# dfm/george

Hardware: AMD Instinct MI355X
Metric: gp_compute_plus_log_likelihood_effective_tflops (higher is better)
Workload: dtype f64; 1 GPU; N=65536 1-D sorted uniform(0,10) x, var(y)*ExpSquaredKernel(1.0), yerr=0.1, dense Cholesky fp64 (BasicSolver path): compute()+log_likelihood(); N=65536, kernel=ExpSquared, solver=dense-cholesky, parallelism=1gpu

## Files before the change

george_amd/_native.py:

```python
import ctypes as C
import os

import numpy as np

_HERE = os.path.dirname(os.path.abspath(__file__))
LIB_PATH = os.path.join(_HERE, "csrc", "libgeorge_amd.so")

GH_MAX_AXES, GH_MAX_NDIM, GH_MAX_PARAMS, GH_MAX_METRIC = 8, 16, 4, 36
GH_MAX_NODES, GH_MAX_GRAD, GH_MAX_STACK = 64, 64, 8
GH_OK, GH_ERR_NOT_PD, GH_ERR_BAD_ARG, GH_ERR_HIP, GH_ERR_NOT_COMPUTED, GH_ERR_DIM, GH_ERR_NOMEM, GH_ERR_RANK, GH_REFACTORIZE = range(9)
GH_OP_LEAF, GH_OP_SUM, GH_OP_PRODUCT = 0, 1, 2


class gh_knode(C.Structure):
    _fields_ = [
        ("op", C.c_int32), ("kernel_type", C.c_int32), ("metric_type", C.c_int32),
        ("ndim", C.c_int32), ("naxes", C.c_int32), ("blocked", C.c_int32),
        ("n_params", C.c_int32), ("n_metric", C.c_int32),
        ("axes", C.c_int32 * GH_MAX_AXES),
        ("params", C.c_double * GH_MAX_PARAMS),
        ("constant", C.c_double),
        ("metric", C.c_double * GH_MAX_METRIC),
        ("min_block", C.c_double * GH_MAX_AXES),
        ("max_block", C.c_double * GH_MAX_AXES),
# ... 63 lines not shown

_vp, _dp, _i64, _i32 = C.c_void_p, C.c_void_p, C.c_int64, C.c_int32

SIGNATURES = {
    "gh_device_count": (C.c_int, []),
    "gh_last_error": (C.c_char_p, []),
    "gh_version": (C.c_char_p, []),
    "gh_release_caches": (None, [C.c_int32]),
    "gh_set_cache_limit": (None, [C.c_int64]),
    "gh_microbench_mfma_f64": (C.c_int, [C.POINTER(C.c_double)]),
    "gh_microbench_hbm_copy": (C.c_int, [C.POINTER(C.c_double)]),
    "gh_debug_set_mfma": (C.c_int, [C.c_int]),
    "gh_debug_set_gemm_sp": (C.c_int, [C.c_int]),
    "gh_debug_set_adaptive_panels": (C.c_int, [C.c_int]),
    "gh_debug_set_update_group": (C.c_int, [C.c_int]),
    "gh_debug_set_update_hide": (C.c_double, [C.c_double]),
    "gh_debug_chol_plan": (C.c_int, [C.c_int64, C.c_int64, C.c_int64, C.c_int32, C.c_double, C.POINTER(C.c_int64), C.c_int32, C.POINTER(C.c_int32),
                                     C.POINTER(C.c_int64), C.c_int32, C.POINTER(C.c_int32), C.POINTER(C.c_int32)]),
    "gh_debug_set_build_on_chain": (C.c_int, [C.c_int]),
    "gh_debug_set_append_path": (C.c_int, [C.c_int]),
    "gh_debug_set_remove_path": (C.c_int, [C.c_int]),
    "gh_debug_check_remove_args": (C.c_int, [_i64, _dp, _i64]),
    "gh_debug_set_gemm_grouped": (C.c_int, [C.c_int]),
    "gh_debug_set_hodlr_passes": (C.c_int, [C.c_int]),
    "gh_debug_set_hodlr_leaf_gj": (C.c_int, [C.c_int]),
    "gh_debug_set_hodlr_wave_aca": (C.c_int, [C.c_int]),
    "gh_debug_set_hodlr_coop_wgs": (C.c_int, [C.c_int]),
    "gh_debug_set_hodlr_coop_lower": (C.c_int, [C.c_int]),
    "gh_debug_set_hodlr_lpt": (C.c_int, [C.c_int]),
    "gh_debug_set_hodlr_u_from_v": (C.c_int, [C.c_int]),
    "gh_debug_set_hodlr_core_fused": (C.c_int, [C.c_int]),
    "gh_debug_set_hodlr_coop_singles": (C.c_int, [C.c_int]),
    "gh_debug_set_hodlr_leaf_fused": (C.c_int, [C.c_int]),
    "gh_debug_set_hodlr_strip_cols": (C.c_int, [C.c_int]),
    "gh_debug_stream_overlap": (C.c_int, [_vp, C.POINTER(C.c_double), C.c_int]),
    "gh_debug_stream_dispatch": (C.c_int, [_vp, C.POINTER(C.c_double), C.c_int]),
    "gh_microbench_suite": (C.c_int, [C.POINTER(C.c_double), C.c_int]),
    "gh_microbench_mfma_f64_ceiling": (C.c_int, [C.POINTER(C.c_double), C.c_int]),
    "gh_kernel_create": (C.c_int, [C.POINTER(gh_knode), C.c_int, C.POINTER(_vp)]),
    "gh_kernel_destroy": (None, [_vp]),
    "gh_kernel_ndim": (C.c_int, [_vp]),
    "gh_kernel_size": (C.c_int, [_vp]),
    "gh_kernel_value_general": (C.c_int, [_vp, _dp, _i64, _dp, _i64, _dp]),
    "gh_kernel_value_symmetric": (C.c_int, [_vp, _dp, _i64, _dp]),
    "gh_kernel_value_diagonal": (C.c_int, [_vp, _dp, _dp, _i64, _dp]),
    "gh_kernel_gradient_general": (C.c_int, [_vp, _dp, _dp, _i64, _dp, _i64, _dp]),
# ... 160 lines not shown
```

george_amd/csrc/gh_chol.hip:

```cpp
#include <math.h>
#include <chrono>
#include "gh_chol_impl.h"
#include "../../include/george_amd_debug.h"

__global__ __launch_bounds__(256) void potf2_inv_kernel(double* A, long lda, double* dinv,
                                                        long long* info, long long base) {
  __shared__ double s[T * LP];
  __shared__ int fail_at;
  const int tid = threadIdx.x;
  if (*info != 0) return;
  if (tid == 0) fail_at = -1;
  for (int idx = tid; idx < T * T; idx += 256) {
    const int i = idx >> 7, j = idx & 127;
    s[i * LP + j] = A[(long)i * lda + j];
  }
  __syncthreads();
  const int ty = tid >> 4, tx = tid & 15;
  for (int j = 0; j < T; ++j) {
    const double d = s[j * LP + j];
    if (!(d > 0.0)) {
      if (tid == 0) fail_at = j;
      break;
    }
    const double ajj = sqrt(d);
// ... 238 lines not shown
  *st = s->st;
  *bufs = s->batch;
  return GH_OK;
}
extern "C" int gh_chol_get_update_intervals(const gh_chol* s, double* out, int32_t max_launches, int32_t* n_out) {
  if (!s || !n_out || (max_launches > 0 && !out)) { gh_set_error("null argument"); return GH_ERR_BAD_ARG; }
  const int32_t have = (int32_t)(s->upd_intervals.size() / 3);
  *n_out = have;
  for (int32_t i = 0; i < have && i < max_launches; ++i)
    for (int q = 0; q < 3; ++q) out[3 * i + q] = s->upd_intervals[3 * (size_t)i + q];
  return GH_OK;
}
extern "C" int gh_chol_get_profile(const gh_chol* s, gh_chol_profile* out) {
  if (!s || !out) { gh_set_error("null argument"); return GH_ERR_BAD_ARG; }
  *out = s->prof;
  return GH_OK;
}

static inline double* blk(double* A, int64_t ld, int64_t r, int64_t c) { return A + r * ld + c; }

static thread_local bool t_gemm_small_lds = false;
struct SmallLdsGuard { bool prev; explicit SmallLdsGuard(bool v) : prev(t_gemm_small_lds) { t_gemm_small_lds = v; } ~SmallLdsGuard() { t_gemm_small_lds = prev; } };
int gh_gemm_nt(hipStream_t st, double* C, int64_t ldc, const double* A, int64_t lda, const double* B, int64_t ldb,
               int64_t M, int64_t N, int64_t K, double alpha, double beta, bool lower) {
  GhGemm g = gemm_desc(C, ldc, A, lda, true, B, ldb, true, M, N, K, alpha, beta);
  g.small_lds = t_gemm_small_lds;
  g.lower = lower;
  return gh_launch_gemm(g, st);
}

static bool use_simple_potf2() {
  static int v = -1;
  if (v < 0) { const char* e = getenv("GEORGE_AMD_POTF2"); v = (e && e[0] == 's') ? 1 : 0; }
  return v == 1;
}

int gh_chol_potrf_block(hipStream_t st, double* A, int64_t ld, int64_t n, double* dinv, long long* d_info, long long base) {
  for (int64_t j0 = 0; j0 < n; j0 += T) {
    double* dj = dinv + (j0 / T) * T * T;
    if (use_simple_potf2()) {
      hipLaunchKernelGGL(potf2_inv_kernel, dim3(1), dim3(256), 0, st, blk(A, ld, j0, j0), (long)ld, dj, d_info, base + j0);
      GH_HIP(hipGetLastError());
    } else {
      GH_CHECK(gh_launch_potf2_mfma(blk(A, ld, j0, j0), ld, dj, d_info, base + j0, st));
    }
    const int64_t rem = n - (j0 + T);
    if (rem > 0) {
      double* P = blk(A, ld, j0 + T, j0);
      GH_CHECK(gh_gemm_nt(st, P, ld, P, ld, dj, T, rem, T, T, 1.0, 0.0, false));
      GH_CHECK(gh_gemm_nt(st, blk(A, ld, j0 + T, j0 + T), ld, P, ld, P, ld, rem, rem, T, -1.0, 1.0, true));
// ... 186 lines not shown
    if (prev) GH_HIP(hipStreamWaitEvent(sp, prev, 0));
    GH_CHECK(narrow(sp, j, j + 1));
    const int last_near = std::min(j + depth, P - 1);
    if (j + 2 <= last_near || (depth >= 2 && j + 2 <= P - 1)) GH_HIP(hipStreamWaitEvent(sn, s->ev_p[j], 0));
    for (int c = j + 2; c <= last_near; ++c) {
      if (c == j + depth && j >= 1) GH_HIP(hipStreamWaitEvent(sn, s->ev_w[j - 1], 0));
      GH_CHECK(narrow(sn, j, c));
      if (c == j + 2) GH_HIP(hipEventRecord(s->ev_nf[j], sn));
    }
    if (depth >= 2 && j + 2 > last_near) GH_HIP(hipEventRecord(s->ev_nf[j], sn));
    const int cw = j + depth + 1;
    hipStream_t sw = wide_stream(j);
    if (sw_prev && sw_prev != sw && j >= 1) GH_HIP(hipStreamWaitEvent(sw, s->ev_w[j - 1], 0));
    sw_prev = sw;
    GH_HIP(hipStreamWaitEvent(sw, s->ev_p[j], 0));
    if (cw <= P - 1) {
      const int64_t kw = c0(cw), m2 = np - kw;
      const long et = prof ? s->next_ev() : -1;
      if (et >= 0) {
        GH_HIP(hipEventRecord(s->ev_pool[et].a, sw)); s->ev_trailing.push_back((size_t)et); s->ev_update.push_back((size_t)et);
        s->ev_update_flops.push_back((double)(m2 / T) * (m2 / T + 1) / 2.0 * 2.0 * T * T * (double)nbc(j));
      }
      const double* P2 = blk(A, ld, kw, c0(j));
      GH_CHECK(gh_gemm_nt(sw, blk(A, ld, kw, kw), ld, P2, ld, P2, ld, m2, m2, nbc(j), -1.0, 1.0, true));
      if (et >= 0) GH_HIP(hipEventRecord(s->ev_pool[et].b, sw));
      const double tiles = (double)(m2 / T) * (m2 / T + 1) / 2.0;
      s->prof.trailing_flops += tiles * 2.0 * T * T * (double)nbc(j);
      s->prof.update_flops += tiles * 2.0 * T * T * (double)nbc(j);
      s->prof.n_trailing += 1;
    }
    GH_HIP(hipEventRecord(s->ev_w[j], sw));
  }
  const bool join_on_chain = !s->shared_streams || gh_shared_main_crowded(s->opts.device);
  if (sm != s->st && join_on_chain) {
    GH_HIP(hipEventRecord(s->ev_sync[2], sn));
    GH_HIP(hipStreamWaitEvent(sp, s->ev_sync[2], 0));
    GH_HIP(hipEventRecord(s->ev_xfer, sm));
    GH_HIP(hipStreamWaitEvent(sp, s->ev_xfer, 0));
    if (P >= 2) GH_HIP(hipStreamWaitEvent(sp, s->ev_w[P - 2], 0));
    s->tail = sp;
    return GH_OK;
  }
  GH_HIP(hipEventRecord(s->ev_sync[1], sp));
  GH_HIP(hipStreamWaitEvent(s->st, s->ev_sync[1], 0));
  GH_HIP(hipEventRecord(s->ev_sync[2], sn));
  GH_HIP(hipStreamWaitEvent(s->st, s->ev_sync[2], 0));
  if (sm != s->st) {
// ... 253 lines not shown
```

george_amd/csrc/gh_chol_impl.h:

```cpp
#pragma once
#include <string.h>
#include <algorithm>
#include <vector>
#include "gh_common.h"
#include "gh_chol_plan.h"

#define T 128
#define LP 129
#define CHAIN_THREADS 512

struct EvPair { hipEvent_t a, b; };

struct gh_chol {
  gh_chol_opts opts;
  hipStream_t st = nullptr;
  hipStream_t st2 = nullptr;
  hipStream_t st3 = nullptr;
  bool shared_streams = false;
  hipStream_t st4 = nullptr;
  hipEvent_t ev_diag[32] = {};
  hipEvent_t ev_aux = nullptr, ev_aux2 = nullptr;
  std::vector<hipEvent_t> ev_p, ev_w, ev_nf;
  GhCholPlan plan;
  std::vector<hipEvent_t> ev_plan;
// ... 54 lines not shown
static inline unsigned* fwd_flags(const gh_chol* s) { return (unsigned*)s->chain.p; }
static inline unsigned* bwd_flags(const gh_chol* s) { return (unsigned*)s->chain.p + (s->np / T + 1); }
static inline int* fwd_fail(const gh_chol* s) { return (int*)(fwd_flags(s) + s->np / T); }
static inline int* bwd_fail(const gh_chol* s) { return (int*)(bwd_flags(s) + s->np / T); }
static inline int* append_fail(const gh_chol* s) { return (int*)s->chain.p; }

static inline int read_scalars(const gh_chol* s, double* host, int count, hipStream_t st) {
  GH_HIP(hipMemcpyAsync(host, s->scal.d(), (size_t)count * sizeof(double), hipMemcpyDeviceToHost, st));
  return GH_OK;
}
static inline long long info_from_bits(double word) { long long info = 0; memcpy(&info, &word, sizeof(long long)); return info; }

static inline GhGemm gemm_desc(double* C, int64_t ldc, const double* A, int64_t lda, bool a_km, const double* B, int64_t ldb, bool b_km,
                               int64_t M, int64_t N, int64_t K, double alpha, double beta) {
  GhGemm g{};
  g.C = C; g.ldc = ldc; g.A = A; g.lda = lda; g.B = B; g.ldb = ldb; g.M = M; g.N = N; g.K = K;
  g.alpha = alpha; g.beta = beta; g.a_km = a_km; g.b_km = b_km;
  return g;
}

int gh_chol_set_device(gh_chol* s);
int gh_chol_need_computed(gh_chol* s);
int gh_gemm_nt(hipStream_t st, double* C, int64_t ldc, const double* A, int64_t lda, const double* B, int64_t ldb,
               int64_t M, int64_t N, int64_t K, double alpha, double beta, bool lower);
int gh_chol_potrf_block(hipStream_t st, double* A, int64_t ld, int64_t n, double* dinv, long long* d_info, long long base);
struct ComputeCtx { long e_all = -1, e_build = -1; };
int gh_chol_compute_enqueue(gh_chol* s, gh_kernel* k, const double* x, int64_t n, int32_t ndim, const double* yerr, ComputeCtx& c);
int gh_chol_compute_finish(gh_chol* s, const ComputeCtx& c, double ld_host, long long info_host, double* logdet_out);

int gh_launch_potf2_mfma(double* A, int64_t lda, double* dinv, long long* info, long long base, hipStream_t st);

int gh_launch_logdet(const double* A, long lda, long n, double* out, double* part, hipStream_t st);
int gh_launch_logdet_accum(const double* A, long lda, long n, double* out, hipStream_t st);
int gh_chol_linv(hipStream_t st, const double* L, const double* dinv, int64_t np, double* Linv);
int gh_launch_trsv_fwd_chain(const double* L, long ld, const double* dinv, int64_t nt, const double* w, double* z, unsigned* flags, hipStream_t st);
int gh_launch_trsv_bwd_chain(const double* L, long ld, const double* dinv, int64_t nt, const double* w, double* x, unsigned* flags, hipStream_t st);
int gh_launch_trsv_fwd_chain_rows(const double* L, long ld, const double* dinv, int64_t nt0, const double* Y, long ldy, double* Z, long ldz,
                                  int64_t m, bool multi, int* fail, hipStream_t st);
int gh_chain_timeout(const char* who, bool forward_failed, bool backward_failed);
```

george_amd/csrc/gh_common.h:

```cpp
#pragma once
#include <hip/hip_runtime.h>
#include <stdint.h>
#include <stdio.h>
#include <functional>
#include <mutex>
#include <string>
#include <vector>
#include "../../include/george_amd.h"
#include "gh_eval.h"

#define GH_TILE 128

void gh_set_error(const char* fmt, ...);

#define GH_HIP(expr)                                                                   \
  do {                                                                                 \
    hipError_t e_ = (expr);                                                            \
    if (e_ != hipSuccess) {                                                            \
      gh_set_error("HIP error %d (%s) at %s:%d: %s", (int)e_, hipGetErrorString(e_),   \
                   __FILE__, __LINE__, #expr);                                         \
      return GH_ERR_HIP;                                                               \
    }                                                                                  \
  } while (0)

// ... 130 lines not shown
int gh_lgo_gram_chunks(int64_t n, int nslots, int64_t* rows_per);
int gh_launch_lgo_gram(const double* Linv, int64_t np, int64_t n, const GhLgoSlots& t, double* part, double* Cs, hipStream_t st);
int gh_launch_lgo_gather(const double* Kinv, int64_t np, const GhLgoSlots& t, double* Cs, hipStream_t st);
int gh_launch_lgo_slots(const double* R, const double* Rinv, const GhLgoSlots& t, const double* alpha, double* resid, double* var,
                        double* u_pt, double* lpd, double* cov, double* Ws, hipStream_t st);
int gh_launch_lgo_block_scale(const double* Kinv, int64_t np, int64_t n, const GhLgoSlots& t, const double* Tm, double* S,
                              hipStream_t st);

int gh_launch_potf2_batched(double* A, int64_t lda, int64_t stride_a, double* dinv, int64_t stride_d, long long* info,
                            int nbatch, hipStream_t st);

struct GhGemm {
  double* C; int64_t ldc;
  const double* A; int64_t lda;
  const double* B; int64_t ldb;
  int64_t M, N, K;
  double alpha, beta;
  bool a_km, b_km;
  bool lower;
  bool klo_max;
  bool khi_col;
  bool khi_row;
  bool small_lds;
  int stair_n = 0;
  int64_t stair_rows = 0;
  const int64_t* stair_cols = nullptr;
};
#define GH_GEMM_STAIR_MAX 128
int gh_launch_gemm(const GhGemm& g, hipStream_t st);

int gh_stage_points(const double* xs, int64_t m, int ndim, GhBuf& own, hipStream_t st, const double** xs_dev);
int gh_copy_rows(double* dst, int64_t ldd, const double* src, int64_t lds, int64_t cols, int64_t rows, bool from_caller, hipStream_t st);
int gh_launch_colreduce(const double* A, const double* z, const double* P, const double* Q, int64_t ld, int64_t nrows, int64_t rows_per,
                        int64_t nchunks, int64_t cols, double* pmu, double* pvar, int64_t ldp, double* mu, double* var, int threads,
                        hipStream_t st);
typedef std::function<int(const double* sK, double* sSecond, int64_t ld, int64_t np, int cw, size_t strip_bytes)> GhMakeSecond;
int gh_predict_strips(gh_kernel* k, const double* x, int64_t n, int ndim, const double* alpha, const double* xs_dev, int64_t m,
                      int64_t strip_cols, int64_t red_rows, int64_t red_chunks, double* mu, double* var, double* cov, hipStream_t st,
                      bool first_second, const GhMakeSecond& make_second);
struct GhPstrf {
  double* A; int64_t lda, stride_a;
  int64_t m, nbatch;
  double tol; const double* tol_dev;
  double* L; int64_t ldl, stride_l;
  int64_t rows_l, cols_l;
  long long* piv; long long* rank;
  double* resid;
  void* work; size_t work_bytes;
};
size_t gh_pstrf_work_bytes(int64_t m, int64_t nbatch);
int gh_launch_pstrf(const GhPstrf& p, hipStream_t st);
struct GhSample {
// ... 19 lines not shown
```

george_amd/csrc/gh_gemm.hip:

```cpp
#include <stdlib.h>
#include <algorithm>
#include "gh_common.h"
#include "../../include/george_amd_debug.h"

#include "gh_gemm_tile.h"

#ifndef GH_GEMM_SP_DEFAULT
#define GH_GEMM_SP_DEFAULT 1
#endif

struct GemmDev {
  double* C; long ldc;
  const double* A; long lda;
  const double* B; long ldb;
  long K;
  double alpha, beta;
  int tiles_m, tiles_n;
  int lower, klo_max, khi_col, khi_row;
  long nblk;
  int preload;
  int prio;
  int grouped;
  int stair_n, stair_h;
  unsigned stair_pre[GH_GEMM_STAIR_MAX + 1];
};

__device__ __forceinline__ long xcd_remap(long bid, long nblk) {
  const long q = nblk / 8, r = nblk % 8;
  const long xcd = bid % 8, idx = bid / 8;
  return (xcd < r ? xcd * (q + 1) : r * (q + 1) + (xcd - r) * q) + idx;
}

#ifndef GH_TILE_GROUP
#define GH_TILE_GROUP 8
#endif
__device__ __forceinline__ void grouped_rect(long l, int rows, int cols, int& tm, int& tn) {
  constexpr int G = GH_TILE_GROUP;
  const int g = (int)(l / ((long)G * cols));
  const int gg = min(G, rows - g * G);
  const long r = l - (long)g * G * cols;
  tn = (int)(r / gg);
  tm = g * G + (int)(r % gg);
}
__device__ __forceinline__ void grouped_tri(long l, int T, int& tm, int& tn) {
  constexpr int G = GH_TILE_GROUP;
  constexpr long H = (long)G * (G + 1) / 2;
  long g = (long)((sqrt(((double)H - 0.5 * G * G) * ((double)H - 0.5 * G * G) + 2.0 * G * G * (double)l) - ((double)H - 0.5 * G * G)) /
                  ((double)G * G));
  auto start = [&](long q) { return (long)G * G * q * (q - 1) / 2 + q * H; };
  while (start(g) > l) --g;
  while (start(g + 1) <= l) ++g;
  const int r0 = (int)g * G, gg = min(G, T - r0);
  long r = l - start(g);
  const long rect = (long)gg * (r0 + 1);
  if (r < rect) {
    tn = (int)(r / gg);
    tm = r0 + (int)(r % gg);
    return;
  }
  r -= rect;
  int j = 1;
  while (r >= gg - j) { r -= gg - j; ++j; }
  tn = r0 + j;
  tm = r0 + j + (int)r;
}
__device__ __forceinline__ bool tile_of(const GemmDev& g, int& tm, int& tn) {
  const bool rowmajor = !g.grouped;
  if (g.stair_n) {
    const long ls = xcd_remap(blockIdx.x, g.nblk);
    int s = 0;
    while (s + 1 < g.stair_n && ls >= (long)g.stair_pre[s + 1]) ++s;
    const int r = (int)(ls - (long)g.stair_pre[s]);
    tn = r / g.stair_h;
    tm = (g.stair_n - 1 - s) * g.stair_h + r % g.stair_h;
    return true;
  }
  const long l = (g.klo_max | g.khi_col | g.khi_row) ? (long)blockIdx.x : xcd_remap(blockIdx.x, g.nblk);
  if (g.lower) {
    const long tri = (long)g.tiles_n * (g.tiles_n + 1) / 2;
    if (l < tri) {
      if (!rowmajor) {
        grouped_tri(l, g.tiles_n, tm, tn);
      } else {
        long t = (long)((sqrt(8.0 * (double)l + 1.0) - 1.0) * 0.5);
        while (t * (t + 1) / 2 > l) --t;
        while ((t + 1) * (t + 2) / 2 <= l) ++t;
        tm = (int)t;
        tn = (int)(l - t * (t + 1) / 2);
      }
    } else if (!rowmajor) {
      grouped_rect(l - tri, g.tiles_m - g.tiles_n, g.tiles_n, tm, tn);
      tm += g.tiles_n;
    } else {
      tm = g.tiles_n + (int)((l - tri) / g.tiles_n);
      tn = (int)((l - tri) % g.tiles_n);
    }
  } else if (!rowmajor) {
    grouped_rect(l, g.tiles_m, g.tiles_n, tm, tn);
  } else {
    tm = (int)(l / g.tiles_n);
    tn = (int)(l % g.tiles_n);
  }
  return true;
}

template <bool KM>
__device__ __forceinline__ void stage_load(const double* base, long ld, long r0, long k0, int tid, double2 (&v)[4]) {
  if (KM) {
    const int row = tid >> 3, kc = (tid & 7) * 2;
#pragma unroll
    for (int i = 0; i < 4; ++i)
      v[i] = *reinterpret_cast<const double2*>(base + (r0 + row + 32 * i) * ld + k0 + kc);
  } else {
    const int k = tid >> 6, m = (tid & 63) * 2;
#pragma unroll
    for (int i = 0; i < 4; ++i)
      v[i] = *reinterpret_cast<const double2*>(base + (k0 + k + 4 * i) * ld + r0 + m);
  }
}
template <bool KM>
__device__ __forceinline__ void stage_store(double* s, int tid, const double2 (&v)[4]) {
  if (KM) {
    const int row = tid >> 3, kc = (tid & 7) * 2;
#pragma unroll
    for (int i = 0; i < 4; ++i)
// ... 112 lines not shown
    for (int i = 0; i < 4; ++i)
#pragma unroll
      for (int j = 0; j < 4; ++j)
        acc[i][j] = __builtin_amdgcn_mfma_f64_16x16x4f64(a[0][i], b[0][j], acc[i][j], 0, 0, 0);
    __builtin_amdgcn_sched_barrier(0);
    if (kt + 1 < nk) {
      if (cur) { GH_DMA_ISSUE(oa, sA[0]) GH_DMA_ISSUE(ob, sB[0]) }
      else     { GH_DMA_ISSUE(oa, sA[1]) GH_DMA_ISSUE(ob, sB[1]) }
    }
    __builtin_amdgcn_sched_barrier(0);
#pragma unroll
    for (int kk = 1; kk < 4; ++kk)
#pragma unroll
      for (int i = 0; i < 4; ++i)
#pragma unroll
        for (int j = 0; j < 4; ++j)
          acc[i][j] = __builtin_amdgcn_mfma_f64_16x16x4f64(a[kk][i], b[kk][j], acc[i][j], 0, 0, 0);
    __builtin_amdgcn_sched_barrier(0);
    __syncthreads();
  }
  gemm_epilogue(g, acc, row0 + wm * 64, col0 + wn * 64, fr, fk);
}

template <bool LOWER>
__global__ __launch_bounds__(256, 2) void gemm_f64_mfma_dma_sp(GemmDev g) {
  __shared__ __attribute__((aligned(1024))) double sm[4 * BM * BK];
  double* const sA0 = sm; double* const sA1 = sm + BM * BK;
  double* const sB0 = sm + 2 * BM * BK; double* const sB1 = sm + 3 * BM * BK;
  int tm, tn;
  if (!tile_of(g, tm, tn)) return;
  if (g.prio) __builtin_amdgcn_s_setprio(3);
  const long row0 = (long)tm * BM, col0 = (long)tn * BN;
  const int tid = threadIdx.x, lane = tid & 63, wave = __builtin_amdgcn_readfirstlane(tid >> 6);
  const int wm = wave >> 1, wn = wave & 1;
  const int fr = lane & 15, fk = lane >> 4;
  v4d acc[4][4];
  const long nk = g.K / BK;
  DmaOperand<true> oa, ob;
  oa.init(g.A, g.lda, row0, 0, wave, lane, wm);
  ob.init(g.B, g.ldb, col0, 0, wave, lane, wn);
  const int dst = wave * 4 * 128;
  const unsigned lbase = (unsigned)(unsigned long)(gh_lds_void*)sm;
  const unsigned pa0 = lbase + (unsigned)(oa.f0 + oa.off2[0]) * 8u, pa1 = lbase + (unsigned)(oa.f0 + oa.off2[1]) * 8u;
  const unsigned pb0 = lbase + 2u * BM * BK * 8u + (unsigned)(ob.f0 + ob.off2[0]) * 8u;
  const unsigned pb1 = lbase + 2u * BM * BK * 8u + (unsigned)(ob.f0 + ob.off2[1]) * 8u;
  constexpr int B1 = BM * BK * 8;
  v2d a01[4], b01[4], a23[4], b23[4];

  GH_DMA_ISSUE(oa, sA0) GH_DMA_ISSUE(ob, sB0)
  gemm_init_acc(g, acc, row0 + wm * 64, col0 + wn * 64, fr, fk);
  __syncthreads();
// ... 283 lines not shown
extern "C" int gh_debug_set_mfma(int mode) {
  const int prev = mfma_mode();
  g_mfma = mode == 0 ? 0 : 1;
  return prev;
}

static int g_gemm_sp = -1;
static int gemm_sp_mode() {
  if (g_gemm_sp < 0) g_gemm_sp = GH_GEMM_SP_DEFAULT;
  return g_gemm_sp;
}
static int g_gemm_grouped = -1;
extern "C" int gh_debug_set_gemm_grouped(int mode) {
  const int prev = g_gemm_grouped;
  g_gemm_grouped = mode < 0 ? -1 : (mode != 0);
  return prev;
}
extern "C" int gh_debug_set_gemm_sp(int mode) {
  const int prev = gemm_sp_mode();
  g_gemm_sp = mode < 0 ? GH_GEMM_SP_DEFAULT : (mode != 0);
  return prev;
}

int gh_launch_gemm(const GhGemm& h, hipStream_t st) {
  if (h.M <= 0 || h.N <= 0) return GH_OK;
  if (h.M % BM || h.N % BN || h.K % BK) { gh_set_error("gemm: sizes must be multiples of the tile (%ld %ld %ld)", (long)h.M, (long)h.N, (long)h.K); return GH_ERR_BAD_ARG; }
  if (h.lower && h.M < h.N) { gh_set_error("gemm: lower needs M >= N (a lower trapezoid: the leading N columns of a lower-triangular C)"); return GH_ERR_BAD_ARG; }
  GemmDev g;
  g.C = h.C; g.ldc = h.ldc; g.A = h.A; g.lda = h.lda; g.B = h.B; g.ldb = h.ldb; g.K = h.K;
  g.alpha = h.alpha; g.beta = h.beta;
  g.tiles_m = (int)(h.M / BM); g.tiles_n = (int)(h.N / BN);
  g.lower = h.lower; g.klo_max = h.klo_max; g.khi_col = h.khi_col; g.khi_row = h.khi_row;
  g.nblk = h.lower ? (long)g.tiles_n * (g.tiles_n + 1) / 2 + (long)(g.tiles_m - g.tiles_n) * g.tiles_n : (long)g.tiles_m * g.tiles_n;
  g.stair_n = 0; g.stair_h = 0;
  if (h.stair_n > 0) {
    g.stair_n = h.stair_n; g.stair_h = (int)(h.stair_rows / BM);
    g.tiles_m = g.stair_n * g.stair_h; g.tiles_n = (int)(h.stair_cols[h.stair_n - 1] / BN);
    long at = 0;
    for (int s = 0; s < h.stair_n; ++s) { g.stair_pre[s] = (unsigned)at; at += (long)g.stair_h * (h.stair_cols[h.stair_n - 1 - s] / BN); }
    g.stair_pre[h.stair_n] = (unsigned)at;
    g.nblk = at;
  }
  g.prio = g.nblk <= 512 ? 1 : 0;
  g.grouped = (!(h.klo_max | h.khi_col | h.khi_row) && (long)h.N * h.K * 8 > (128L << 20)) ? 1 : 0;
  if (g_gemm_grouped >= 0 && !(h.klo_max | h.khi_col | h.khi_row)) g.grouped = g_gemm_grouped;
  g.preload = (h.beta != 0.0 && (h.beta == h.alpha || h.beta == -h.alpha)) ? 1 : 0;
  if (g.nblk > 0x7fffffffL) { gh_set_error("gemm: grid too large"); return GH_ERR_BAD_ARG; }
  const dim3 grid((unsigned)g.nblk), block(256);
  const int mode = mfma_mode();
#define GH_GEMM_LAUNCH(AK, BKM) hipLaunchKernelGGL((gemm_f64_valu<AK, BKM>), grid, block, 0, st, g)
  constexpr int64_t GH_DMA_MAX_LD = ((1LL << 31) - 4096) / (128 * 8);
  const bool dma = mode == 1 && h.lda % 2 == 0 && h.ldb % 2 == 0 && h.lda <= GH_DMA_MAX_LD && h.ldb <= GH_DMA_MAX_LD &&
                   ((uintptr_t)h.A % 16) == 0 && ((uintptr_t)h.B % 16) == 0;
#define GH_DMA_LAUNCH(AK, BKM)                                                                            \
  do {                                                                                                   \
    if (h.lower) hipLaunchKernelGGL((gemm_f64_mfma_dma<AK, BKM, true>), grid, block, 0, st, g);          \
    else         hipLaunchKernelGGL((gemm_f64_mfma_dma<AK, BKM, false>), grid, block, 0, st, g);         \
  } while (0)
  const bool inplace = (const double*)h.C == h.A || (const double*)h.C == h.B;
  if (dma && !h.stair_n && h.a_km && h.b_km && h.K == 128 && g.nblk <= 128 && !h.klo_max && !h.khi_col && !h.khi_row && !h.small_lds &&
      (!inplace || ((const double*)h.C == h.A && (const double*)h.C != h.B && h.N == 128 && !h.lower))) {
    GemmDev q = g;
    if (inplace) {
      q.tiles_m = (int)(h.M / 16); q.tiles_n = 1;
      q.nblk = q.tiles_m;
      hipLaunchKernelGGL((gemm_f64_mfma_k128<1, 4, 1, 2>), dim3((unsigned)q.nblk), block, 0, st, q);
    } else {
      q.tiles_m = (int)(h.M / 64); q.tiles_n = (int)(h.N / 64);
      q.nblk = (long)q.tiles_m * q.tiles_n;
      hipLaunchKernelGGL((gemm_f64_mfma_k128<2, 2, 2, 2>), dim3((unsigned)q.nblk), block, 0, st, q);
    }
    GH_HIP(hipGetLastError());
    return GH_OK;
  }
  if (dma && !h.stair_n && h.a_km && h.b_km && g.nblk <= 128 && !h.klo_max && !h.khi_col && !h.khi_row && (!h.lower || h.M == h.N) &&
      (!inplace || (h.N == 128 && !h.lower))) {
    GemmDev q = g;
    if (inplace) {
      q.tiles_m = (int)(h.M / 64); q.tiles_n = 1;
      q.nblk = q.tiles_m;
      hipLaunchKernelGGL(gemm_f64_mfma_dma64<4>, dim3((unsigned)q.nblk), block, 0, st, q);
    } else {
      q.tiles_m = (int)(h.M / 64); q.tiles_n = (int)(h.N / 64);
      q.nblk = h.lower ? 4 * g.nblk : (long)q.tiles_m * q.tiles_n;
      hipLaunchKernelGGL(gemm_f64_mfma_dma64<2>, dim3((unsigned)q.nblk), block, 0, st, q);
    }
  }
  else if (dma && h.a_km && h.b_km && gemm_sp_mode() && !h.klo_max && !h.khi_col && !h.khi_row && h.K % (2 * BK) == 0) {
    if (h.lower) hipLaunchKernelGGL(gemm_f64_mfma_dma_sp<true>, grid, block, 0, st, g);
    else         hipLaunchKernelGGL(gemm_f64_mfma_dma_sp<false>, grid, block, 0, st, g);
  }
  else if (dma && h.a_km && h.b_km)   GH_DMA_LAUNCH(true, true);
  else if (dma && h.a_km && !h.b_km)  GH_DMA_LAUNCH(true, false);
  else if (dma && !h.a_km && !h.b_km) GH_DMA_LAUNCH(false, false);
  else if (dma)                       GH_DMA_LAUNCH(false, true);
#undef GH_DMA_LAUNCH
  else if (h.a_km && h.b_km) GH_GEMM_LAUNCH(true, true);
  else if (h.a_km && !h.b_km) GH_GEMM_LAUNCH(true, false);
  else if (!h.a_km && !h.b_km) GH_GEMM_LAUNCH(false, false);
  else GH_GEMM_LAUNCH(false, true);
#undef GH_GEMM_LAUNCH
  GH_HIP(hipGetLastError());
  return GH_OK;
}

extern "C" int gh_dev_gemm_nt_stair(double* c, int64_t ldc, const double* a, int64_t lda, const double* b, int64_t ldb,
                                    int64_t group_rows, int32_t n_groups, const int64_t* group_cols, int64_t k, void* stream) {
  if (n_groups <= 0) return GH_OK;
  if (!group_cols || group_rows <= 0 || group_rows % BM) { gh_set_error("gemm_nt_stair: group_rows must be a positive multiple of 128"); return GH_ERR_BAD_ARG; }
  long tiles = 0;
  for (int g = 0; g < n_groups; ++g) {
    if (group_cols[g] <= 0 || group_cols[g] % BN || (g > 0 && group_cols[g] < group_cols[g - 1])) {
      gh_set_error("gemm_nt_stair: group_cols must be positive multiples of 128, non-decreasing"); return GH_ERR_BAD_ARG; }
// ... 250 lines not shown
```

include/george_amd_debug.h:

```cpp
#ifndef GEORGE_AMD_DEBUG_H_
#define GEORGE_AMD_DEBUG_H_

#include "george_amd.h"

#ifdef __cplusplus
extern "C" {
#endif

int gh_microbench_mfma_f64(double* tflops_out);
int gh_debug_set_mfma(int mode);
int gh_debug_set_gemm_sp(int mode);
int gh_debug_set_gemm_grouped(int mode);
int gh_debug_set_build_on_chain(int on);
int gh_debug_set_append_path(int path);
int gh_debug_set_remove_path(int path);
int gh_debug_check_remove_args(int64_t n, const int64_t* idx, int64_t m);
int gh_debug_set_adaptive_panels(int on);
int gh_debug_set_update_group(int gmax);
double gh_debug_set_update_hide(double hide);
int gh_debug_chol_plan(int64_t np, int64_t nb, int64_t bound, int32_t gmax, double hide, int64_t* panel_starts_out, int32_t max_starts,
                       int32_t* n_starts, int64_t* ops_out, int32_t max_ops, int32_t* n_ops, int32_t* n_events);
int gh_debug_set_hodlr_passes(int mask);
int gh_debug_set_hodlr_leaf_gj(int on);
int gh_debug_set_hodlr_wave_aca(int on);
int gh_debug_set_hodlr_coop_wgs(int n);
int gh_debug_set_hodlr_coop_lower(int div);
int gh_debug_set_hodlr_lpt(int on);
int gh_debug_set_hodlr_u_from_v(int on);
int gh_debug_set_hodlr_core_fused(int on);
int gh_debug_set_hodlr_coop_singles(int on);
int gh_debug_set_hodlr_leaf_fused(int on);
int gh_debug_set_hodlr_strip_cols(int cols);
int gh_debug_stream_overlap(gh_chol* s, double* out, int n);
int gh_debug_stream_dispatch(gh_chol* s, double* out, int n);
int gh_microbench_hbm_copy(double* gbps_out);
// ... 14 lines not shown
```

Baseline: 73.33 TFLOP/s.

## Split GEMM wave-quantization tail tiles into quarter tiles to fill idle CUs

```diff
diff --git a/george_amd/_native.py b/george_amd/_native.py
--- a/george_amd/_native.py
+++ b/george_amd/_native.py
@@ -109,6 +109,8 @@
     "gh_debug_set_remove_path": (C.c_int, [C.c_int]),
     "gh_debug_check_remove_args": (C.c_int, [_i64, _dp, _i64]),
     "gh_debug_set_gemm_grouped": (C.c_int, [C.c_int]),
+    "gh_debug_set_gemm_tail": (C.c_int, [C.c_int, C.c_int]),
+    "gh_debug_gemm_tail_map": (C.c_int, [_i32, _i32, _i32, _i32, _i64, C.POINTER(C.c_int32), _i64, C.POINTER(C.c_int64)]),
     "gh_debug_set_hodlr_passes": (C.c_int, [C.c_int]),
     "gh_debug_set_hodlr_leaf_gj": (C.c_int, [C.c_int]),
     "gh_debug_set_hodlr_wave_aca": (C.c_int, [C.c_int]),
diff --git a/george_amd/csrc/gh_chol.hip b/george_amd/csrc/gh_chol.hip
--- a/george_amd/csrc/gh_chol.hip
+++ b/george_amd/csrc/gh_chol.hip
@@ -284,10 +284,11 @@
 static thread_local bool t_gemm_small_lds = false;
 struct SmallLdsGuard { bool prev; explicit SmallLdsGuard(bool v) : prev(t_gemm_small_lds) { t_gemm_small_lds = v; } ~SmallLdsGuard() { t_gemm_small_lds = prev; } };
 int gh_gemm_nt(hipStream_t st, double* C, int64_t ldc, const double* A, int64_t lda, const double* B, int64_t ldb,
-               int64_t M, int64_t N, int64_t K, double alpha, double beta, bool lower) {
+               int64_t M, int64_t N, int64_t K, double alpha, double beta, bool lower, int cus) {
   GhGemm g = gemm_desc(C, ldc, A, lda, true, B, ldb, true, M, N, K, alpha, beta);
   g.small_lds = t_gemm_small_lds;
   g.lower = lower;
+  g.cus = cus;
   return gh_launch_gemm(g, st);
 }
 
@@ -520,7 +521,8 @@
         s->ev_update_flops.push_back((double)(m2 / T) * (m2 / T + 1) / 2.0 * 2.0 * T * T * (double)nbc(j));
       }
       const double* P2 = blk(A, ld, kw, c0(j));
-      GH_CHECK(gh_gemm_nt(sw, blk(A, ld, kw, kw), ld, P2, ld, P2, ld, m2, m2, nbc(j), -1.0, 1.0, true));
+      GH_CHECK(gh_gemm_nt(sw, blk(A, ld, kw, kw), ld, P2, ld, P2, ld, m2, m2, nbc(j), -1.0, 1.0, true,
+                          sw == s->st ? 0 : gh_device_cus() - s->mask_reserved));
       if (et >= 0) GH_HIP(hipEventRecord(s->ev_pool[et].b, sw));
       const double tiles = (double)(m2 / T) * (m2 / T + 1) / 2.0;
       s->prof.trailing_flops += tiles * 2.0 * T * T * (double)nbc(j);
diff --git a/george_amd/csrc/gh_chol_impl.h b/george_amd/csrc/gh_chol_impl.h
--- a/george_amd/csrc/gh_chol_impl.h
+++ b/george_amd/csrc/gh_chol_impl.h
@@ -100,7 +100,7 @@
 int gh_chol_set_device(gh_chol* s);
 int gh_chol_need_computed(gh_chol* s);
 int gh_gemm_nt(hipStream_t st, double* C, int64_t ldc, const double* A, int64_t lda, const double* B, int64_t ldb,
-               int64_t M, int64_t N, int64_t K, double alpha, double beta, bool lower);
+               int64_t M, int64_t N, int64_t K, double alpha, double beta, bool lower, int cus = 0);
 int gh_chol_potrf_block(hipStream_t st, double* A, int64_t ld, int64_t n, double* dinv, long long* d_info, long long base);
 struct ComputeCtx { long e_all = -1, e_build = -1; };
 int gh_chol_compute_enqueue(gh_chol* s, gh_kernel* k, const double* x, int64_t n, int32_t ndim, const double* yerr, ComputeCtx& c);
diff --git a/george_amd/csrc/gh_common.h b/george_amd/csrc/gh_common.h
--- a/george_amd/csrc/gh_common.h
+++ b/george_amd/csrc/gh_common.h
@@ -176,12 +176,14 @@
   bool khi_col;
   bool khi_row;
   bool small_lds;
+  int cus = 0;
   int stair_n = 0;
   int64_t stair_rows = 0;
   const int64_t* stair_cols = nullptr;
 };
 #define GH_GEMM_STAIR_MAX 128
 int gh_launch_gemm(const GhGemm& g, hipStream_t st);
+int gh_device_cus();
 
 int gh_stage_points(const double* xs, int64_t m, int ndim, GhBuf& own, hipStream_t st, const double** xs_dev);
 int gh_copy_rows(double* dst, int64_t ldd, const double* src, int64_t lds, int64_t cols, int64_t rows, bool from_caller, hipStream_t st);
diff --git a/george_amd/csrc/gh_gemm.hip b/george_amd/csrc/gh_gemm.hip
--- a/george_amd/csrc/gh_gemm.hip
+++ b/george_amd/csrc/gh_gemm.hip
@@ -4,6 +4,7 @@
 #include "../../include/george_amd_debug.h"
 
 #include "gh_gemm_tile.h"
+#include "gh_gemm_tail.h"
 
 #ifndef GH_GEMM_SP_DEFAULT
 #define GH_GEMM_SP_DEFAULT 1
@@ -18,6 +19,7 @@
   int tiles_m, tiles_n;
   int lower, klo_max, khi_col, khi_row;
   long nblk;
+  long nbig;
   int preload;
   int prio;
   int grouped;
@@ -25,49 +27,9 @@
   unsigned stair_pre[GH_GEMM_STAIR_MAX + 1];
 };
 
-__device__ __forceinline__ long xcd_remap(long bid, long nblk) {
-  const long q = nblk / 8, r = nblk % 8;
-  const long xcd = bid % 8, idx = bid / 8;
-  return (xcd < r ? xcd * (q + 1) : r * (q + 1) + (xcd - r) * q) + idx;
-}
-
-#ifndef GH_TILE_GROUP
-#define GH_TILE_GROUP 8
-#endif
-__device__ __forceinline__ void grouped_rect(long l, int rows, int cols, int& tm, int& tn) {
-  constexpr int G = GH_TILE_GROUP;
-  const int g = (int)(l / ((long)G * cols));
-  const int gg = min(G, rows - g * G);
-  const long r = l - (long)g * G * cols;
-  tn = (int)(r / gg);
-  tm = g * G + (int)(r % gg);
-}
-__device__ __forceinline__ void grouped_tri(long l, int T, int& tm, int& tn) {
-  constexpr int G = GH_TILE_GROUP;
-  constexpr long H = (long)G * (G + 1) / 2;
-  long g = (long)((sqrt(((double)H - 0.5 * G * G) * ((double)H - 0.5 * G * G) + 2.0 * G * G * (double)l) - ((double)H - 0.5 * G * G)) /
-                  ((double)G * G));
-  auto start = [&](long q) { return (long)G * G * q * (q - 1) / 2 + q * H; };
-  while (start(g) > l) --g;
-  while (start(g + 1) <= l) ++g;
-  const int r0 = (int)g * G, gg = min(G, T - r0);
-  long r = l - start(g);
-  const long rect = (long)gg * (r0 + 1);
-  if (r < rect) {
-    tn = (int)(r / gg);
-    tm = r0 + (int)(r % gg);
-    return;
-  }
-  r -= rect;
-  int j = 1;
-  while (r >= gg - j) { r -= gg - j; ++j; }
-  tn = r0 + j;
-  tm = r0 + j + (int)r;
-}
 __device__ __forceinline__ bool tile_of(const GemmDev& g, int& tm, int& tn) {
-  const bool rowmajor = !g.grouped;
   if (g.stair_n) {
-    const long ls = xcd_remap(blockIdx.x, g.nblk);
+    const long ls = gh_xcd_remap(blockIdx.x, g.nblk);
     int s = 0;
     while (s + 1 < g.stair_n && ls >= (long)g.stair_pre[s + 1]) ++s;
     const int r = (int)(ls - (long)g.stair_pre[s]);
@@ -75,32 +37,8 @@
     tm = (g.stair_n - 1 - s) * g.stair_h + r % g.stair_h;
     return true;
   }
-  const long l = (g.klo_max | g.khi_col | g.khi_row) ? (long)blockIdx.x : xcd_remap(blockIdx.x, g.nblk);
-  if (g.lower) {
-    const long tri = (long)g.tiles_n * (g.tiles_n + 1) / 2;
-    if (l < tri) {
-      if (!rowmajor) {
-        grouped_tri(l, g.tiles_n, tm, tn);
-      } else {
-        long t = (long)((sqrt(8.0 * (double)l + 1.0) - 1.0) * 0.5);
-        while (t * (t + 1) / 2 > l) --t;
-        while ((t + 1) * (t + 2) / 2 <= l) ++t;
-        tm = (int)t;
-        tn = (int)(l - t * (t + 1) / 2);
-      }
-    } else if (!rowmajor) {
-      grouped_rect(l - tri, g.tiles_m - g.tiles_n, g.tiles_n, tm, tn);
-      tm += g.tiles_n;
-    } else {
-      tm = g.tiles_n + (int)((l - tri) / g.tiles_n);
-      tn = (int)((l - tri) % g.tiles_n);
-    }
-  } else if (!rowmajor) {
-    grouped_rect(l, g.tiles_m, g.tiles_n, tm, tn);
-  } else {
-    tm = (int)(l / g.tiles_n);
-    tn = (int)(l % g.tiles_n);
-  }
+  const long l = (g.klo_max | g.khi_col | g.khi_row) ? (long)blockIdx.x : gh_xcd_remap(blockIdx.x, g.nblk);
+  gh_tile_at(g.tiles_m, g.tiles_n, g.lower, g.grouped, l, tm, tn);
   return true;
 }
 
@@ -259,11 +197,123 @@
   gemm_epilogue(g, acc, row0 + wm * 64, col0 + wn * 64, fr, fk);
 }
 
+__device__ __forceinline__ void gemm_quarter_tile(const GemmDev& g, double* sm, long row0, long col0, int wave, int lane) {
+  double* const sA = sm;
+  double* const sB = sm + 2 * 64 * BK;
+  const int wm = wave >> 1, wn = wave & 1;
+  const int fr = lane & 15, fk = lane >> 4;
+  const long nk = g.K / BK;
+  const double* ga[2];
+  const double* gb[2];
+#pragma unroll
+  for (int i = 0; i < 2; ++i) {
+    const int r = wave * 16 + i * 8 + (lane >> 3);
+    const int piece = ((lane & 7) ^ ((r >> 1) & 7)) * 2;
+    ga[i] = g.A + (row0 + r) * g.lda + piece;
+    gb[i] = g.B + (col0 + r) * g.ldb + piece;
+  }
+  const int sw = (fr >> 1) & 7;
+  int offk[4];
+#pragma unroll
+  for (int kk = 0; kk < 4; ++kk) offk[kk] = GH_KM_OFFK(kk, fk, sw);
+  const int rowA = (wm * 32 + fr) * BK, rowB = (wn * 32 + fr) * BK;
+  const int dst = wave * 2 * 128;
+#define GH_QUARTER_ISSUE(buf)                                                                                    \
+  _Pragma("unroll") for (int i = 0; i < 2; ++i) {                                                                \
+    __builtin_amdgcn_global_load_lds((gh_glb_void*)ga[i], (gh_lds_void*)(sA + (buf) * 64 * BK + dst + i * 128), 16, 0, 0); \
+    ga[i] += BK;                                                                                                 \
+  }                                                                                                              \
+  _Pragma("unroll") for (int i = 0; i < 2; ++i) {                                                                \
+    __builtin_amdgcn_global_load_lds((gh_glb_void*)gb[i], (gh_lds_void*)(sB + (buf) * 64 * BK + dst + i * 128), 16, 0, 0); \
+    gb[i] += BK;                                                                                                 \
+  }
+  v4d acc[2][2];
+  const double alpha = g.alpha;
+  double* cbase = g.C + (row0 + wm * 32 + fk) * g.ldc + col0 + wn * 32 + fr;
+  GH_QUARTER_ISSUE(0)
+  if (g.preload) {
+    const double rho = (g.beta == g.alpha) ? 1.0 : -1.0;
+#pragma unroll
+    for (int i = 0; i < 2; ++i)
+#pragma unroll
+      for (int r = 0; r < 4; ++r)
+#pragma unroll
+        for (int j = 0; j < 2; ++j) acc[i][j][r] = rho * cbase[(long)(i * 16 + 4 * r) * g.ldc + j * 16];
+  } else {
+#pragma unroll
+    for (int i = 0; i < 2; ++i)
+#pragma unroll
+      for (int j = 0; j < 2; ++j) acc[i][j] = (v4d){0.0, 0.0, 0.0, 0.0};
+  }
+  __syncthreads();
+  for (long kt = 0; kt < nk; ++kt) {
+    const int cur = (int)(kt & 1);
+    const double* pa = sA + cur * 64 * BK + rowA;
+    const double* pb = sB + cur * 64 * BK + rowB;
+    double a[4][2], b[4][2];
+#pragma unroll
+    for (int kk = 0; kk < 4; ++kk) {
+#pragma unroll
+      for (int i = 0; i < 2; ++i) a[kk][i] = pa[i * 16 * BK + offk[kk]];
+#pragma unroll
+      for (int j = 0; j < 2; ++j) b[kk][j] = pb[j * 16 * BK + offk[kk]];
+    }
+    __builtin_amdgcn_sched_barrier(0);
+    if (kt + 1 < nk) {
+      if (cur) { GH_QUARTER_ISSUE(0) } else { GH_QUARTER_ISSUE(1) }
+    }
+    __builtin_amdgcn_sched_barrier(0);
+#pragma unroll
+    for (int kk = 0; kk < 4; ++kk)
+#pragma unroll
+      for (int i = 0; i < 2; ++i)
+#pragma unroll
+        for (int j = 0; j < 2; ++j)
+          acc[i][j] = __builtin_amdgcn_mfma_f64_16x16x4f64(a[kk][i], b[kk][j], acc[i][j], 0, 0, 0);
+    __builtin_amdgcn_sched_barrier(0);
+    __syncthreads();
+  }
+#undef GH_QUARTER_ISSUE
+  const double beta = g.preload ? 0.0 : g.beta;
+  if (beta == 0.0) {
+#pragma unroll
+    for (int i = 0; i < 2; ++i)
+#pragma unroll
+      for (int r = 0; r < 4; ++r)
+#pragma unroll
+        for (int j = 0; j < 2; ++j) cbase[(long)(i * 16 + 4 * r) * g.ldc + j * 16] = alpha * acc[i][j][r];
+  } else {
+    double c[2][4][2];
+#pragma unroll
+    for (int i = 0; i < 2; ++i)
+#pragma unroll
+      for (int r = 0; r < 4; ++r)
+#pragma unroll
+        for (int j = 0; j < 2; ++j) c[i][r][j] = cbase[(long)(i * 16 + 4 * r) * g.ldc + j * 16];
+#pragma unroll
+    for (int i = 0; i < 2; ++i)
+#pragma unroll
+      for (int r = 0; r < 4; ++r)
+#pragma unroll
+        for (int j = 0; j < 2; ++j)
+          cbase[(long)(i * 16 + 4 * r) * g.ldc + j * 16] = fma(beta, c[i][r][j], alpha * acc[i][j][r]);
+  }
+}
+
 template <bool LOWER>
 __global__ __launch_bounds__(256, 2) void gemm_f64_mfma_dma_sp(GemmDev g) {
   __shared__ __attribute__((aligned(1024))) double sm[4 * BM * BK];
   double* const sA0 = sm; double* const sA1 = sm + BM * BK;
   double* const sB0 = sm + 2 * BM * BK; double* const sB1 = sm + 3 * BM * BK;
+  if ((long)blockIdx.x >= g.nbig) {
+    long t; int q, qm, qn;
+    gh_tail_quarter(g.nblk, g.nblk - g.nbig, (long)blockIdx.x - g.nbig, t, q);
+    gh_tile_at(g.tiles_m, g.tiles_n, g.lower, g.grouped, gh_xcd_remap(t, g.nblk), qm, qn);
+    if (g.prio) __builtin_amdgcn_s_setprio(3);
+    gemm_quarter_tile(g, sm, (long)qm * BM + (q >> 1) * 64, (long)qn * BN + (q & 1) * 64,
+                      __builtin_amdgcn_readfirstlane(threadIdx.x >> 6), threadIdx.x & 63);
+    return;
+  }
   int tm, tn;
   if (!tile_of(g, tm, tn)) return;
   if (g.prio) __builtin_amdgcn_s_setprio(3);
@@ -593,6 +643,53 @@
   return prev;
 }
 
+#ifndef GH_GEMM_TAIL_E
+#define GH_GEMM_TAIL_E 0.65
+#endif
+static int g_gemm_tail = 1, g_gemm_tail_slots = 0;
+extern "C" int gh_debug_set_gemm_tail(int mode, int slots) {
+  const int prev = g_gemm_tail;
+  g_gemm_tail = (mode == 0 || mode == 2) ? mode : 1;
+  g_gemm_tail_slots = slots > 0 ? slots : 0;
+  return prev;
+}
+int gh_device_cus() {
+  static int cus[64] = {0};
+  int dev = 0;
+  if (hipGetDevice(&dev) != hipSuccess) { (void)hipGetLastError(); return 256; }
+  if (dev < 0 || dev >= 64) return 256;
+  if (!cus[dev]) {
+    hipDeviceProp_t prop;
+    cus[dev] = (hipGetDeviceProperties(&prop, dev) == hipSuccess && prop.multiProcessorCount > 0) ? prop.multiProcessorCount : 256;
+  }
+  return cus[dev];
+}
+static long gemm_tail_tiles(const GhGemm& h, long nblk, bool inplace) {
+  if (g_gemm_tail == 0 || h.stair_n || inplace) return 0;
+  if (g_gemm_tail == 2) return std::min<long>(nblk, g_gemm_tail_slots);
+  if (nblk <= 128) return 0;
+  const long S = 2L * (h.cus > 0 ? h.cus : gh_device_cus());
+  const long r = nblk % S;
+  if (nblk <= S || r == 0 || (double)r >= GH_GEMM_TAIL_E * (double)S) return 0;
+  return std::min(nblk, (r + 7) & ~7L);
+}
+extern "C" int gh_debug_gemm_tail_map(int32_t tiles_m, int32_t tiles_n, int32_t lower, int32_t grouped, int64_t nt, int32_t* out,
+                                      int64_t max_rows, int64_t* n_rows) {
+  if (tiles_m <= 0 || tiles_n <= 0 || (lower && tiles_m < tiles_n) || !n_rows || (max_rows > 0 && !out)) {
+    gh_set_error("gemm_tail_map: tile counts must be positive (lower: tiles_m >= tiles_n)"); return GH_ERR_BAD_ARG; }
+  GhTileOrder o;
+  o.tiles_m = tiles_m; o.tiles_n = tiles_n; o.lower = lower != 0; o.grouped = grouped != 0;
+  o.nblk = gh_tile_count(tiles_m, tiles_n, o.lower);
+  if (nt < 0 || nt > o.nblk) { gh_set_error("gemm_tail_map: the tail must be 0 .. %ld tiles", o.nblk); return GH_ERR_BAD_ARG; }
+  *n_rows = gh_tail_grid(o.nblk, nt);
+  for (int64_t b = 0; b < *n_rows && b < max_rows; ++b) {
+    int tm, tn, q;
+    gh_tail_map(o, nt, b, tm, tn, q);
+    out[3 * b] = tm; out[3 * b + 1] = tn; out[3 * b + 2] = q;
+  }
+  return GH_OK;
+}
+
 int gh_launch_gemm(const GhGemm& h, hipStream_t st) {
   if (h.M <= 0 || h.N <= 0) return GH_OK;
   if (h.M % BM || h.N % BN || h.K % BK) { gh_set_error("gemm: sizes must be multiples of the tile (%ld %ld %ld)", (long)h.M, (long)h.N, (long)h.K); return GH_ERR_BAD_ARG; }
@@ -603,6 +700,7 @@
   g.tiles_m = (int)(h.M / BM); g.tiles_n = (int)(h.N / BN);
   g.lower = h.lower; g.klo_max = h.klo_max; g.khi_col = h.khi_col; g.khi_row = h.khi_row;
   g.nblk = h.lower ? (long)g.tiles_n * (g.tiles_n + 1) / 2 + (long)(g.tiles_m - g.tiles_n) * g.tiles_n : (long)g.tiles_m * g.tiles_n;
+  g.nbig = g.nblk;
   g.stair_n = 0; g.stair_h = 0;
   if (h.stair_n > 0) {
     g.stair_n = h.stair_n; g.stair_h = (int)(h.stair_rows / BM);
@@ -610,7 +708,7 @@
     long at = 0;
     for (int s = 0; s < h.stair_n; ++s) { g.stair_pre[s] = (unsigned)at; at += (long)g.stair_h * (h.stair_cols[h.stair_n - 1 - s] / BN); }
     g.stair_pre[h.stair_n] = (unsigned)at;
-    g.nblk = at;
+    g.nblk = g.nbig = at;
   }
   g.prio = g.nblk <= 512 ? 1 : 0;
   g.grouped = (!(h.klo_max | h.khi_col | h.khi_row) && (long)h.N * h.K * 8 > (128L << 20)) ? 1 : 0;
@@ -629,7 +727,10 @@
     else         hipLaunchKernelGGL((gemm_f64_mfma_dma<AK, BKM, false>), grid, block, 0, st, g);         \
   } while (0)
   const bool inplace = (const double*)h.C == h.A || (const double*)h.C == h.B;
-  if (dma && !h.stair_n && h.a_km && h.b_km && h.K == 128 && g.nblk <= 128 && !h.klo_max && !h.khi_col && !h.khi_row && !h.small_lds &&
+  const bool sp = dma && h.a_km && h.b_km && gemm_sp_mode() && !h.klo_max && !h.khi_col && !h.khi_row && h.K % (2 * BK) == 0;
+  const long nt = sp ? gemm_tail_tiles(h, g.nblk, inplace) : 0;
+  const bool forced = nt > 0 && g_gemm_tail == 2;
+  if (!forced && dma && !h.stair_n && h.a_km && h.b_km && h.K == 128 && g.nblk <= 128 && !h.klo_max && !h.khi_col && !h.khi_row && !h.small_lds &&
       (!inplace || ((const double*)h.C == h.A && (const double*)h.C != h.B && h.N == 128 && !h.lower))) {
     GemmDev q = g;
     if (inplace) {
@@ -644,7 +745,7 @@
     GH_HIP(hipGetLastError());
     return GH_OK;
   }
-  if (dma && !h.stair_n && h.a_km && h.b_km && g.nblk <= 128 && !h.klo_max && !h.khi_col && !h.khi_row && (!h.lower || h.M == h.N) &&
+  if (!forced && dma && !h.stair_n && h.a_km && h.b_km && g.nblk <= 128 && !h.klo_max && !h.khi_col && !h.khi_row && (!h.lower || h.M == h.N) &&
       (!inplace || (h.N == 128 && !h.lower))) {
     GemmDev q = g;
     if (inplace) {
@@ -657,9 +758,12 @@
       hipLaunchKernelGGL(gemm_f64_mfma_dma64<2>, dim3((unsigned)q.nblk), block, 0, st, q);
     }
   }
-  else if (dma && h.a_km && h.b_km && gemm_sp_mode() && !h.klo_max && !h.khi_col && !h.khi_row && h.K % (2 * BK) == 0) {
-    if (h.lower) hipLaunchKernelGGL(gemm_f64_mfma_dma_sp<true>, grid, block, 0, st, g);
-    else         hipLaunchKernelGGL(gemm_f64_mfma_dma_sp<false>, grid, block, 0, st, g);
+  else if (sp) {
+    g.nbig = g.nblk - nt;
+    if (gh_tail_grid(g.nblk, nt) > 0x7fffffffL) { gh_set_error("gemm: grid too large"); return GH_ERR_BAD_ARG; }
+    const dim3 grid_sp((unsigned)gh_tail_grid(g.nblk, nt));
+    if (h.lower) hipLaunchKernelGGL(gemm_f64_mfma_dma_sp<true>, grid_sp, block, 0, st, g);
+    else         hipLaunchKernelGGL(gemm_f64_mfma_dma_sp<false>, grid_sp, block, 0, st, g);
   }
   else if (dma && h.a_km && h.b_km)   GH_DMA_LAUNCH(true, true);
   else if (dma && h.a_km && !h.b_km)  GH_DMA_LAUNCH(true, false);
diff --git a/george_amd/csrc/gh_gemm_tail.h b/george_amd/csrc/gh_gemm_tail.h
--- /dev/null
+++ b/george_amd/csrc/gh_gemm_tail.h
@@ -0,0 +1,105 @@
+#ifndef GH_GEMM_TAIL_H_
+#define GH_GEMM_TAIL_H_
+#include <math.h>
+
+#if defined(__HIPCC__) || defined(__CUDACC__)
+#define GH_HD __host__ __device__ __forceinline__
+#else
+#define GH_HD static inline
+#endif
+
+#ifndef GH_TILE_GROUP
+#define GH_TILE_GROUP 8
+#endif
+
+struct GhTileOrder {
+  int tiles_m, tiles_n;
+  int lower;
+  int grouped;
+  long nblk;
+};
+GH_HD long gh_tile_count(int tiles_m, int tiles_n, int lower) {
+  return lower ? (long)tiles_n * (tiles_n + 1) / 2 + (long)(tiles_m - tiles_n) * tiles_n : (long)tiles_m * tiles_n;
+}
+
+GH_HD long gh_xcd_remap(long bid, long nblk) {
+  const long q = nblk / 8, r = nblk % 8;
+  const long xcd = bid % 8, idx = bid / 8;
+  return (xcd < r ? xcd * (q + 1) : r * (q + 1) + (xcd - r) * q) + idx;
+}
+
+GH_HD void gh_grouped_rect(long l, int rows, int cols, int& tm, int& tn) {
+  const int G = GH_TILE_GROUP;
+  const int g = (int)(l / ((long)G * cols));
+  const int gg = G < rows - g * G ? G : rows - g * G;
+  const long r = l - (long)g * G * cols;
+  tn = (int)(r / gg);
+  tm = g * G + (int)(r % gg);
+}
+GH_HD void gh_grouped_tri(long l, int T, int& tm, int& tn) {
+  const int G = GH_TILE_GROUP;
+  const long H = (long)G * (G + 1) / 2;
+  long g = (long)((sqrt(((double)H - 0.5 * G * G) * ((double)H - 0.5 * G * G) + 2.0 * G * G * (double)l) - ((double)H - 0.5 * G * G)) /
+                  ((double)G * G));
+  while ((long)G * G * g * (g - 1) / 2 + g * H > l) --g;
+  while ((long)G * G * (g + 1) * g / 2 + (g + 1) * H <= l) ++g;
+  const int r0 = (int)g * G, gg = G < T - r0 ? G : T - r0;
+  long r = l - ((long)G * G * g * (g - 1) / 2 + g * H);
+  const long rect = (long)gg * (r0 + 1);
+  if (r < rect) {
+    tn = (int)(r / gg);
+    tm = r0 + (int)(r % gg);
+    return;
+  }
+  r -= rect;
+  int j = 1;
+  while (r >= gg - j) { r -= gg - j; ++j; }
+  tn = r0 + j;
+  tm = r0 + j + (int)r;
+}
+GH_HD void gh_tile_at(int tiles_m, int tiles_n, int lower, int grouped, long l, int& tm, int& tn) {
+  if (lower) {
+    const long tri = (long)tiles_n * (tiles_n + 1) / 2;
+    if (l < tri) {
+      if (grouped) {
+        gh_grouped_tri(l, tiles_n, tm, tn);
+      } else {
+        long t = (long)((sqrt(8.0 * (double)l + 1.0) - 1.0) * 0.5);
+        while (t * (t + 1) / 2 > l) --t;
+        while ((t + 1) * (t + 2) / 2 <= l) ++t;
+        tm = (int)t;
+        tn = (int)(l - t * (t + 1) / 2);
+      }
+    } else if (grouped) {
+      gh_grouped_rect(l - tri, tiles_m - tiles_n, tiles_n, tm, tn);
+      tm += tiles_n;
+    } else {
+      tm = tiles_n + (int)((l - tri) / tiles_n);
+      tn = (int)((l - tri) % tiles_n);
+    }
+  } else if (grouped) {
+    gh_grouped_rect(l, tiles_m, tiles_n, tm, tn);
+  } else {
+    tm = (int)(l / tiles_n);
+    tn = (int)(l % tiles_n);
+  }
+}
+
+GH_HD long gh_tail_grid(long nblk, long nt) { return nblk + 3 * nt; }
+GH_HD void gh_tail_quarter(long nblk, long nt, long w, long& t, int& q) {
+  const long whole = nt / 8 * 32;
+  if (w < whole) {
+    t = (nblk - nt) + (w & 7) + 8 * (w >> 5);
+    q = (int)((w >> 3) & 3);
+  } else {
+    t = (nblk - nt) + whole / 4 + ((w - whole) >> 2);
+    q = (int)((w - whole) & 3);
+  }
+}
+GH_HD void gh_tail_map(const GhTileOrder& o, long nt, long bid, int& tm, int& tn, int& q) {
+  long t = bid;
+  q = -1;
+  if (bid >= o.nblk - nt) gh_tail_quarter(o.nblk, nt, bid - (o.nblk - nt), t, q);
+  gh_tile_at(o.tiles_m, o.tiles_n, o.lower, o.grouped, gh_xcd_remap(t, o.nblk), tm, tn);
+}
+#endif
diff --git a/include/george_amd_debug.h b/include/george_amd_debug.h
--- a/include/george_amd_debug.h
+++ b/include/george_amd_debug.h
@@ -11,6 +11,9 @@
 int gh_debug_set_mfma(int mode);
 int gh_debug_set_gemm_sp(int mode);
 int gh_debug_set_gemm_grouped(int mode);
+int gh_debug_set_gemm_tail(int mode, int slots);
+int gh_debug_gemm_tail_map(int32_t tiles_m, int32_t tiles_n, int32_t lower, int32_t grouped, int64_t nt, int32_t* out, int64_t max_rows,
+                           int64_t* n_rows);
 int gh_debug_set_build_on_chain(int on);
 int gh_debug_set_append_path(int path);
 int gh_debug_set_remove_path(int path);
```

Result: no change. 73.45 TFLOP/s (median of 6 runs) (+0.2%).
